# AaronZ345/StyleSinger

Hardware: NVIDIA H100
Metric: mel_frames_per_sec_ph2wav_T100 (higher is better)
Workload: dtype f32

## Files before the change

stylesinger_b200/csrc/conv_gemm_tc.cu:

```cuda
#include <cuda_fp16.h>
#include <stdlib.h>
#include <string.h>

#include <atomic>
#include <mutex>
#include <unordered_map>

#include "conv_gemm_tc.cuh"
#include "tc_common.cuh"

namespace ssb {

namespace {

constexpr int BM = 128, BK = 64;
constexpr int A_TILE = BM * BK * 2;
constexpr int EPI_WARPS = 8;
constexpr int NTHREADS = 128 + 32 * EPI_WARPS;
constexpr int XPOSE_BYTES = EPI_WARPS * 32 * 32 * 4;

constexpr int HALO = 8;
constexpr int A3_ROWS = BM + 2 * HALO;
constexpr int A3_TILE = A3_ROWS * BK * 2;
constexpr int ASLOTS = 2;

template <int BN, bool REUSE>
struct Cfg {
  static constexpr int B_TILE = BN * BK * 2;
  static constexpr int STAGE = REUSE ? 2 * B_TILE : 2 * A_TILE + 2 * B_TILE;
  static constexpr int STAGES = BN == 128 ? 3 : 4;
  static constexpr int ARING = REUSE ? ASLOTS * 2 * A3_TILE : 0;
  static constexpr int SMEM = ARING + STAGES * STAGE + XPOSE_BYTES + 1024 + 256;
  static_assert(SMEM <= 227 * 1024, "exceeds the 227 KB of shared memory a Hopper block can have");
};

struct TCParams {
  const int2* tiles;
  int ntiles, NT, taps, kchunks, dil, center, N;
  EpiTC e;
};

using namespace tc;


struct Pre {
  float4 a[8];
};

template <int MODE>
__device__ __forceinline__ void prefetch_chunk(const EpiTC& e, int64_t r0, int nrows, int n, int lane, Pre& p, int tq) {
  (void)nrows;
  if (e.n_valid > 0 && n >= e.n_valid) return;
  const int rq = lane >> 3, q4 = (lane & 7) * 4;
  const float* src = nullptr;
  int64_t st = 0;
  bool once = false;
  if constexpr (MODE == EPI_GENERIC) {
    if (!e.res) return;
    src = e.res + (r0 + rq) * e.ld_res + n + q4; st = 4 * (int64_t)e.ld_res;
  } else if constexpr (MODE == EPI_RES_SKIP) {
    if (n < e.C) {
      if (e.rh) {
        const __half* ph = e.rh + (r0 + rq) * e.ld_rh + n + q4;
        const __half* pl = e.rl + (r0 + rq) * e.ld_rh + n + q4;
        const int64_t sth = 4 * (int64_t)e.ld_rh;
#pragma unroll
        for (int i = 0; i < 8; ++i, ph += sth, pl += sth) {
          const uint2 h = *reinterpret_cast<const uint2*>(ph);
          const uint2 l = *reinterpret_cast<const uint2*>(pl);
          p.a[i] = make_float4(__uint_as_float(h.x), __uint_as_float(h.y), __uint_as_float(l.x), __uint_as_float(l.y));
        }
        return;
      }
      src = e.res + (r0 + rq) * e.ld_res + n + q4; st = 4 * (int64_t)e.ld_res;
    } else if (!e.skip_init) {
      if (e.skip_tiled) {
        src = e.skip + ((int64_t)tq * (e.C >> 5) + ((n - e.C) >> 5)) * 1024 + rq * 32 + q4; st = 128;
      } else {
        src = e.skip + (r0 + rq) * e.ld_skip + (n - e.C) + q4; st = 4 * (int64_t)e.ld_skip;
      }
      once = true;
    } else return;
  } else {
    if (!e.add) return;
    src = e.add + (r0 + rq) * e.ld_add + n + q4; st = 4 * (int64_t)e.ld_add;
    once = true;
  }
  if (once) {
#pragma unroll
    for (int i = 0; i < 8; ++i, src += st) p.a[i] = __ldcs(reinterpret_cast<const float4*>(src));
  } else {
#pragma unroll
    for (int i = 0; i < 8; ++i, src += st) p.a[i] = *reinterpret_cast<const float4*>(src);
  }
}

__device__ __forceinline__ void split_pack4(float a, float b, float c, float d, uint2& uh, uint2& ul) {
  const __half2 h0 = __floats2half2_rn(a, b), h1 = __floats2half2_rn(c, d);
  const float2 f0 = __half22float2(h0), f1 = __half22float2(h1);
  const __half2 l0 = __floats2half2_rn(a - f0.x, b - f0.y), l1 = __floats2half2_rn(c - f1.x, d - f1.y);
  uh.x = *reinterpret_cast<const uint32_t*>(&h0); uh.y = *reinterpret_cast<const uint32_t*>(&h1);
  ul.x = *reinterpret_cast<const uint32_t*>(&l0); ul.y = *reinterpret_cast<const uint32_t*>(&l1);
}
__device__ __forceinline__ void split_pack2(float a, float b, uint32_t& uh, uint32_t& ul) {
  const __half2 h0 = __floats2half2_rn(a, b);
  const float2 f0 = __half22float2(h0);
  const __half2 l0 = __floats2half2_rn(a - f0.x, b - f0.y);
  uh = *reinterpret_cast<const uint32_t*>(&h0);
  ul = *reinterpret_cast<const uint32_t*>(&l0);
}
__device__ __forceinline__ float act_slope_of(int act, float slope) {
  return act == ACT_RELU ? 0.0f : (act == ACT_LRELU ? slope : 1.0f);
}
template <int MODE>
__device__ __forceinline__ void epilogue_chunk(const EpiTC& e, const float4* xb, int64_t r0, int nrows, int n, int lane,
                                               const Pre& pre, int tq) {
  if (e.n_valid > 0 && n >= e.n_valid) return;
  const int q = lane & 7, rq = lane >> 3;
  const int n4 = n + 4 * q;
  const int64_t rb = r0 + rq;
  const float4* xr = xb + rq * 8;
  const int qx = q ^ rq;
  float b0 = 0.f, b1 = 0.f, b2 = 0.f, b3 = 0.f;
  if (e.bias) {
    const float4 bv = __ldg(reinterpret_cast<const float4*>(e.bias + n4));
    b0 = bv.x; b1 = bv.y; b2 = bv.z; b3 = bv.w;
  }
  const int nsteps = nrows > rq ? (nrows - rq + 3) >> 2 : 0;
  if constexpr (MODE == EPI_GATE) {
    const int64_t st = 4 * (int64_t)e.ldh;
    __half* ph = e.oh + rb * e.ldh + (n4 >> 1);
    __half* pl = e.ol + rb * e.ldh + (n4 >> 1);
    const bool has_add = e.add != nullptr;
#pragma unroll
    for (int i = 0; i < 8; ++i, ph += st, pl += st) {
      const float4 acc = xr[i * 32 + (qx ^ (4 * (i & 1)))];
      float g0 = acc.x + b0, f0 = acc.y + b1, g1 = acc.z + b2, f1 = acc.w + b3;
      if (has_add) {
        const float4 ad = pre.a[i];
        g0 += ad.x; f0 += ad.y; g1 += ad.z; f1 += ad.w;
      }
      uint32_t zh, zl;
      split_pack2(gate_act(g0, f0), gate_act(g1, f1), zh, zl);
      if (i < nsteps) {
        *reinterpret_cast<uint32_t*>(ph) = zh;
        *reinterpret_cast<uint32_t*>(pl) = zl;
      }
    }
  } else if constexpr (MODE == EPI_RES_SKIP) {
    if (n < e.C) {
      const float beta = e.beta;
      float s0 = 0.f, s1 = 0.f, s2 = 0.f, s3 = 0.f;
      const bool planes = e.oh != nullptr;
      if (planes && e.vec2) {
        const float4 sv = __ldg(reinterpret_cast<const float4*>(e.vec2 + n4));
        s0 = sv.x; s1 = sv.y; s2 = sv.z; s3 = sv.w;
      }
      const bool res_planes = e.rh != nullptr, has_out = e.out != nullptr;
      float c0 = 0.f, c1 = 0.f, c2 = 0.f, c3 = 0.f;
      if (res_planes && e.vec1) {
        const float4 cv = __ldg(reinterpret_cast<const float4*>(e.vec1 + n4));
        c0 = cv.x; c1 = cv.y; c2 = cv.z; c3 = cv.w;
      }
      float* po = has_out ? e.out + rb * e.ldo + n4 : nullptr;
      const int64_t sto = 4 * (int64_t)e.ldo, sth = 4 * (int64_t)e.ldh;
      __half* ph = planes ? e.oh + rb * e.ldh + n4 : nullptr;
      __half* pl = planes ? e.ol + rb * e.ldh + n4 : nullptr;
#pragma unroll
      for (int i = 0; i < 8; ++i) {
        const float4 acc = xr[i * 32 + (qx ^ (4 * (i & 1)))];
        float4 x0 = pre.a[i];
        if (res_planes) {
          const uint32_t u0 = __float_as_uint(x0.x), u1 = __float_as_uint(x0.y), u2 = __float_as_uint(x0.z), u3 = __float_as_uint(x0.w);
          const float2 h01 = __half22float2(*reinterpret_cast<const __half2*>(&u0)), h23 = __half22float2(*reinterpret_cast<const __half2*>(&u1));
          const float2 l01 = __half22float2(*reinterpret_cast<const __half2*>(&u2)), l23 = __half22float2(*reinterpret_cast<const __half2*>(&u3));
          x0 = make_float4((h01.x + l01.x) - c0, (h01.y + l01.y) - c1, (h23.x + l23.x) - c2, (h23.y + l23.y) - c3);
        }
        const float v0 = (acc.x + b0 + x0.x) * beta, v1 = (acc.y + b1 + x0.y) * beta;
        const float v2 = (acc.z + b2 + x0.z) * beta, v3 = (acc.w + b3 + x0.w) * beta;
        uint2 yh, yl;
        split_pack4(v0 + s0, v1 + s1, v2 + s2, v3 + s3, yh, yl);
        const bool ok = i < nsteps;
        if (ok && has_out) *reinterpret_cast<float4*>(po) = make_float4(v0, v1, v2, v3);
        if (ok && planes) {
          *reinterpret_cast<uint2*>(ph) = yh;
          *reinterpret_cast<uint2*>(pl) = yl;
        }
        po += sto; ph += sth; pl += sth;
      }
    } else {
      const int sc = n4 - e.C;
      const bool init = e.skip_init != 0;
      const bool planes = e.sh != nullptr;
      float* ps = e.skip_tiled ? e.skip + ((int64_t)tq * (e.C >> 5) + ((n - e.C) >> 5)) * 1024 + rq * 32 + 4 * q
                               : e.skip + rb * e.ld_skip + sc;
      const int64_t sts = e.skip_tiled ? 128 : 4 * (int64_t)e.ld_skip, sth = 4 * (int64_t)e.C;
      __half* ph = planes ? e.sh + rb * e.C + sc : nullptr;
      __half* pl = planes ? e.sl + rb * e.C + sc : nullptr;
#pragma unroll
      for (int i = 0; i < 8; ++i) {
        const float4 acc = xr[i * 32 + (qx ^ (4 * (i & 1)))];
        float v0 = acc.x + b0, v1 = acc.y + b1, v2 = acc.z + b2, v3 = acc.w + b3;
        if (!init) {
          const float4 o = pre.a[i];
          v0 += o.x; v1 += o.y; v2 += o.z; v3 += o.w;
        }
        const bool ok = i < nsteps;
        if (ok) __stcs(reinterpret_cast<float4*>(ps), make_float4(v0, v1, v2, v3));
        if (planes) {
          uint2 kh, kl;
          split_pack4(v0, v1, v2, v3, kh, kl);
          if (ok) {
            *reinterpret_cast<uint2*>(ph) = kh;
            *reinterpret_cast<uint2*>(pl) = kl;
          }
        }
        ps += sts; ph += sth; pl += sth;
      }
    }
  } else {
    const float sa = act_slope_of(e.act, e.act_slope), sp = act_slope_of(e.plane_act, e.plane_slope);
    const bool gelu = e.act == ACT_GELU;
    const float alpha = e.alpha;
    const float* rmask = e.rowmask ? e.rowmask + rb : nullptr;
    const bool has_res = e.res != nullptr, has_out = e.out != nullptr, accum = e.accum != 0, planes = e.oh != nullptr;
    const float gamma = e.gamma;
    float s0 = 0.f, s1 = 0.f, s2 = 0.f, s3 = 0.f;
    if (planes && e.vec2) {
      const float4 sv = __ldg(reinterpret_cast<const float4*>(e.vec2 + n4));
      s0 = sv.x; s1 = sv.y; s2 = sv.z; s3 = sv.w;
    }
    float* po = has_out ? e.out + rb * e.ldo + n4 : nullptr;
    int64_t sto = 4 * (int64_t)e.ldo;
    const int64_t sth = 4 * (int64_t)e.ldh;
    if (has_out && e.out_nb > 0) {
      const int blk = n4 / e.out_nb;
      po = e.out + (int64_t)blk * e.out_bs + rb * e.out_nb + (n4 - blk * e.out_nb);
      sto = 4 * (int64_t)e.out_nb;
    }
    __half* ph = planes ? e.oh + rb * e.ldh + n4 : nullptr;
    __half* pl = planes ? e.ol + rb * e.ldh + n4 : nullptr;
    float4 oacc[8];
    if (has_out && accum) {
      const float* pr = po;
#pragma unroll
      for (int i = 0; i < 8; ++i, pr += sto) oacc[i] = *reinterpret_cast<const float4*>(pr);
    }
#pragma unroll
    for (int i = 0; i < 8; ++i) {
      const float4 acc = xr[i * 32 + (qx ^ (4 * (i & 1)))];
      float v0 = (acc.x + b0) * alpha, v1 = (acc.y + b1) * alpha, v2 = (acc.z + b2) * alpha, v3 = (acc.w + b3) * alpha;
      if (gelu) {
        v0 = gelu_erf(v0); v1 = gelu_erf(v1); v2 = gelu_erf(v2); v3 = gelu_erf(v3);
      } else {
        v0 = fmaxf(v0, v0 * sa); v1 = fmaxf(v1, v1 * sa); v2 = fmaxf(v2, v2 * sa); v3 = fmaxf(v3, v3 * sa);
      }
      if (has_res) {
        const float4 x0 = pre.a[i];
        v0 += x0.x; v1 += x0.y; v2 += x0.z; v3 += x0.w;
      }
      if (rmask) {
        const float mk = rmask[4 * i];
        v0 *= mk; v1 *= mk; v2 *= mk; v3 *= mk;
      }
      if (has_out && accum) {
        const float4 o = oacc[i];
        v0 = (v0 + o.x) * gamma; v1 = (v1 + o.y) * gamma; v2 = (v2 + o.z) * gamma; v3 = (v3 + o.w) * gamma;
      }
      const bool ok = i < nsteps;
      if (ok && has_out) *reinterpret_cast<float4*>(po) = make_float4(v0, v1, v2, v3);
      if (planes) {
        const float w0 = v0 + s0, w1 = v1 + s1, w2 = v2 + s2, w3 = v3 + s3;
        uint2 qh, ql;
        split_pack4(fmaxf(w0, w0 * sp), fmaxf(w1, w1 * sp), fmaxf(w2, w2 * sp), fmaxf(w3, w3 * sp), qh, ql);
        if (ok) {
          *reinterpret_cast<uint2*>(ph) = qh;
          *reinterpret_cast<uint2*>(pl) = ql;
        }
      }
      po += sto; ph += sth; pl += sth;
    }
  }
}

template <int BN, int CL, int MODE, bool REUSE>
__global__ void __launch_bounds__(NTHREADS, 1)
conv_gemm_wg_kernel(const __grid_constant__ CUtensorMap tmA_hi, const __grid_constant__ CUtensorMap tmA_lo,
                    const __grid_constant__ CUtensorMap tmB_hi, const __grid_constant__ CUtensorMap tmB_lo,
                    const TCParams p) {
  using K = Cfg<BN, REUSE>;
  constexpr int STAGES = K::STAGES;
  constexpr int HB = BN / CL;
  constexpr int NCH = BN / 32;
  extern __shared__ uint8_t smem_raw[];
  uint8_t* smem = reinterpret_cast<uint8_t*>((reinterpret_cast<uintptr_t>(smem_raw) + 1023) & ~uintptr_t(1023));
  float* xpose = reinterpret_cast<float*>(smem + K::ARING + STAGES * K::STAGE);
  uint64_t* bars = reinterpret_cast<uint64_t*>(smem + K::ARING + STAGES * K::STAGE + XPOSE_BYTES);
  const uint32_t abase = smem_u32(smem), sbase = abase + K::ARING;
  const uint32_t full0 = smem_u32(bars), empty0 = full0 + 8 * STAGES, afull0 = empty0 + 8 * STAGES, aempty0 = afull0 + 8 * ASLOTS;
  const int warp = threadIdx.x >> 5, lane = threadIdx.x & 31;
  const uint32_t rank = CL > 1 ? cluster_rank() : 0u;
  const int cid = (int)blockIdx.x / CL, ncl = (int)gridDim.x / CL;

  if (threadIdx.x == 0) {
    for (int s = 0; s < STAGES; ++s) {
      mbar_init(full0 + 8 * s, 1);
      mbar_init(empty0 + 8 * s, CL * EPI_WARPS);
    }
    for (int s = 0; s < ASLOTS; ++s) {
      mbar_init(afull0 + 8 * s, 1);
      mbar_init(aempty0 + 8 * s, EPI_WARPS);
    }
    asm volatile("fence.mbarrier_init.release.cluster;" ::: "memory");
  }
  if (CL > 1) cluster_sync_all();
  else __syncthreads();

  const int total = (CL > 1 ? (p.ntiles + 1) / 2 : p.ntiles) * p.NT;
  const int nk = p.taps * p.kchunks;

  if (warp < 4) {
    asm volatile("setmaxnreg.dec.sync.aligned.u32 40;\n" ::: "memory");
    if (warp == 0 && lane == 0) {
      int stage = 0, as = 0;
      uint32_t phase = 0, aph = 0;
      auto load_b = [&](const CUtensorMap* mb_h, const CUtensorMap* mb_l, int c0, int brow, uint32_t extra_bytes) {
        mbar_wait(empty0 + 8 * stage, phase ^ 1);
        const uint32_t fb = full0 + 8 * stage;
        mbar_expect_tx(fb, 2 * K::B_TILE + extra_bytes);
        const uint32_t sb = sbase + stage * K::STAGE + (REUSE ? 0u : (uint32_t)(2 * A_TILE));
        if (CL > 1) {
          const uint32_t boff = rank * (uint32_t)(HB * BK * 2);
          tma_load_2d_mc(sb + boff, mb_h, fb, c0, brow + (int)rank * HB, (uint16_t)3);
          tma_load_2d_mc(sb + K::B_TILE + boff, mb_l, fb, c0, brow + (int)rank * HB, (uint16_t)3);
        } else {
          tma_load_2d(sb, mb_h, fb, c0, brow);
          tma_load_2d(sb + K::B_TILE, mb_l, fb, c0, brow);
        }
        return fb;
      };
      for (int tile = cid; tile < total; tile += ncl) {
        const int mq = tile / p.NT, nt = tile - mq * p.NT;
        int mt = CL * mq + (int)rank;
        if (mt >= p.ntiles) mt = CL * mq;
        const int row0 = p.tiles[mt].x;
        if constexpr (REUSE) {
          for (int kc = 0; kc < p.kchunks; ++kc) {
            mbar_wait(aempty0 + 8 * as, aph ^ 1);
            const uint32_t ab = afull0 + 8 * as, sa = abase + as * (2 * A3_TILE);
            mbar_expect_tx(ab, 2 * A3_TILE);
            tma_load_2d(sa, &tmA_hi, ab, kc * BK, row0 - HALO);
            tma_load_2d(sa + A3_TILE, &tmA_lo, ab, kc * BK, row0 - HALO);
            if (++as == ASLOTS) { as = 0; aph ^= 1; }
            for (int tap = 0; tap < 3; ++tap) {
              load_b(&tmB_hi, &tmB_lo, kc * BK, tap * p.N + nt * BN, 0u);
              if (++stage == STAGES) { stage = 0; phase ^= 1; }
            }
          }
        } else {
          for (int kb = 0; kb < nk; ++kb) {
            const int tap = kb / p.kchunks;
            const int c0 = (kb - tap * p.kchunks) * BK;
            const int arow = row0 + (tap - p.center) * p.dil;
            const uint32_t fb = load_b(&tmB_hi, &tmB_lo, c0, tap * p.N + nt * BN, (uint32_t)(2 * A_TILE));
            const uint32_t sa = sbase + stage * K::STAGE;
            tma_load_2d(sa, &tmA_hi, fb, c0, arow);
            tma_load_2d(sa + A_TILE, &tmA_lo, fb, c0, arow);
            if (++stage == STAGES) { stage = 0; phase ^= 1; }
          }
        }
      }
    }
    __syncwarp();
  } else {
    asm volatile("setmaxnreg.inc.sync.aligned.u32 232;\n" ::: "memory");
    const int cw = (warp - 4) >> 2;
    const int ew = (warp - 4) >> 1;
    const int eg = warp & 1;
    float* xb_pair = xpose + ew * 2048;
    const uint32_t pair_bar = 1u + (uint32_t)ew;
    const uint32_t peer_empty0 = CL > 1 ? mapa_u32(empty0, rank ^ 1u) : 0u;
    int stage = 0, as = 0;
    uint32_t phase = 0, aph = 0;
    float acc[BN / 2];
    auto release_b = [&](int st) {
      __syncwarp();
      if (lane == 0) {
        mbar_arrive(empty0 + 8 * st);
        if (CL > 1) mbar_arrive_cluster(peer_empty0 + 8 * st);
      }
    };
    auto mma_block = [&](uint64_t dah, uint64_t dal, uint64_t dbh, uint64_t dbl) {
      wg_fence();
      fence_acc(acc);
#pragma unroll
      for (int ks = 0; ks < BK / 16; ++ks) {
        const uint64_t off = (uint64_t)((ks * 32) >> 4);
        if constexpr (BN == 128) {
          wgmma_n128(acc, dah + off, dbh + off, 1u);
          wgmma_n128(acc, dah + off, dbl + off, 1u);
          wgmma_n128(acc, dal + off, dbh + off, 1u);
        } else {
          wgmma_n64(acc, dah + off, dbh + off, 1u);
          wgmma_n64(acc, dah + off, dbl + off, 1u);
          wgmma_n64(acc, dal + off, dbh + off, 1u);
        }
      }
      wg_commit();
      fence_acc(acc);
      wg_wait<1>();
      fence_acc(acc);
    };
    for (int tile = cid; tile < total; tile += ncl) {
      const int mq = tile / p.NT, nt = tile - mq * p.NT;
      const int mt = CL * mq + (int)rank;
      const int2 t = mt < p.ntiles ? p.tiles[mt] : make_int2(0, 0);
      const int64_t r0 = (int64_t)t.x + ew * 32;
      const int nrows = min(32, max(0, t.y - ew * 32));
      const int tq = mt * 4 + ew;
      const int n0 = nt * BN;
      Pre cur, nxt;
      if (nrows > 0) prefetch_chunk<MODE>(p.e, r0, nrows, n0 + eg * 32, lane, cur, tq);
#pragma unroll
      for (int i = 0; i < BN / 2; ++i) acc[i] = 0.f;
      int prev = -1;
      if constexpr (REUSE) {
        for (int kc = 0; kc < p.kchunks; ++kc) {
          mbar_wait(afull0 + 8 * as, aph);
          const uint32_t sa = abase + as * (2 * A3_TILE) + cw * 8192;
          for (int tap = 0; tap < 3; ++tap) {
            mbar_wait(full0 + 8 * stage, phase);
            const uint32_t sb = sbase + stage * K::STAGE;
            const uint32_t sh = (uint32_t)(HALO + (tap - 1) * p.dil) * 128u;
            mma_block(make_sdesc(sa + sh), make_sdesc(sa + A3_TILE + sh), make_sdesc(sb), make_sdesc(sb + K::B_TILE));
            if (prev >= 0) release_b(prev);
            prev = stage;
            if (++stage == STAGES) { stage = 0; phase ^= 1; }
          }
          wg_wait<0>();
          fence_acc(acc);
          release_b(prev);
          prev = -1;
          __syncwarp();
          if (lane == 0) mbar_arrive(aempty0 + 8 * as);
          if (++as == ASLOTS) { as = 0; aph ^= 1; }
        }
      } else {
        for (int kb = 0; kb < nk; ++kb) {
          mbar_wait(full0 + 8 * stage, phase);
          const uint32_t sa = sbase + stage * K::STAGE;
          mma_block(make_sdesc(sa + cw * 8192), make_sdesc(sa + A_TILE + cw * 8192), make_sdesc(sa + 2 * A_TILE),
                    make_sdesc(sa + 2 * A_TILE + K::B_TILE));
          if (prev >= 0) release_b(prev);
          prev = stage;
          if (++stage == STAGES) { stage = 0; phase ^= 1; }
        }
        wg_wait<0>();
        fence_acc(acc);
        if (prev >= 0) release_b(prev);
      }
      const int rbase = 16 * (warp & 1) + (lane >> 2);
#pragma unroll
      for (int cp = 0; cp < BN / 64; ++cp) {
#pragma unroll
        for (int nb = 0; nb < 8; ++nb) {
          float* xb = xb_pair + (nb >> 2) * 1024;
          const int cc = 8 * (nb & 3) + 2 * (lane & 3);
#pragma unroll
          for (int h = 0; h < 2; ++h) {
            const int rr = rbase + 8 * h;
            const int j = 4 * (8 * cp + nb) + 2 * h;
            *reinterpret_cast<float2*>(xb + (rr * 8 + ((cc >> 2) ^ (rr & 7))) * 4 + (cc & 3)) = make_float2(acc[j], acc[j + 1]);
          }
        }
        named_sync(pair_bar, 64);
        const int ch = 2 * cp + eg;
        if (ch + 2 < NCH && nrows > 0) prefetch_chunk<MODE>(p.e, r0, nrows, n0 + (ch + 2) * 32, lane, nxt, tq);
        if (nrows > 0)
          epilogue_chunk<MODE>(p.e, reinterpret_cast<float4*>(xb_pair + eg * 1024), r0, nrows, n0 + ch * 32, lane, cur, tq);
        cur = nxt;
        named_sync(pair_bar, 64);
      }
    }
  }
  if (CL > 1) cluster_sync_all();
}

__global__ void k_split_planes(const float* x, int ld, int64_t rows, int C, float scale, __half* hi, __half* lo) {
  const int64_t i = (int64_t)blockIdx.x * blockDim.x + threadIdx.x;
  if (i >= rows * C) return;
  const int64_t r = i / C;
  const int c = (int)(i - r * C);
  const float v = x[r * ld + c] * scale;
  const __half h = __float2half_rn(v);
  hi[i] = h;
  lo[i] = __float2half_rn(v - __half2float(h));
}

typedef CUresult (*EncodeTiledFn)(CUtensorMap*, CUtensorMapDataType, cuuint32_t, void*, const cuuint64_t*, const cuuint64_t*,
                                  const cuuint32_t*, const cuuint32_t*, CUtensorMapInterleave, CUtensorMapSwizzle,
                                  CUtensorMapL2promotion, CUtensorMapFloatOOBfill);
std::mutex g_host_mu;

EncodeTiledFn get_encode() {
  static std::atomic<EncodeTiledFn> fn_cached{nullptr};
  static std::atomic<bool> tried{false};
  if (!tried.load(std::memory_order_acquire)) {
    std::lock_guard<std::mutex> lk(g_host_mu);
    if (!tried.load(std::memory_order_relaxed)) {
      void* fn = nullptr;
      cudaDriverEntryPointQueryResult q;
      if (cudaGetDriverEntryPoint("cuTensorMapEncodeTiled", &fn, cudaEnableDefault, &q) == cudaSuccess &&
          q == cudaDriverEntryPointSuccess)
        fn_cached.store((EncodeTiledFn)fn, std::memory_order_relaxed);
      tried.store(true, std::memory_order_release);
    }
  }
  return fn_cached.load(std::memory_order_relaxed);
}

int make_map(CUtensorMap* m, const void* ptr, uint64_t rows, uint64_t cols, uint32_t box_rows) {
  EncodeTiledFn enc = get_encode();
  SSB_CHECK(enc != nullptr, "cuTensorMapEncodeTiled unavailable");
  cuuint64_t dims[2] = {cols, rows};
  cuuint64_t strides[1] = {cols * sizeof(__half)};
  cuuint32_t box[2] = {(cuuint32_t)BK, box_rows};
  cuuint32_t es[2] = {1, 1};
  CUresult rc = enc(m, CU_TENSOR_MAP_DATA_TYPE_FLOAT16, 2, const_cast<void*>(ptr), dims, strides, box, es,
                    CU_TENSOR_MAP_INTERLEAVE_NONE, CU_TENSOR_MAP_SWIZZLE_128B, CU_TENSOR_MAP_L2_PROMOTION_L2_256B,
                    CU_TENSOR_MAP_FLOAT_OOB_FILL_NONE);
  SSB_CHECK(rc == CUDA_SUCCESS, "cuTensorMapEncodeTiled failed");
  return 0;
}

struct MapKey {
  const void* ptr; uint64_t rows; uint32_t cols, box;
  bool operator==(const MapKey& o) const { return ptr == o.ptr && rows == o.rows && cols == o.cols && box == o.box; }
};
struct MapKeyHash {
  size_t operator()(const MapKey& k) const {
    uint64_t h = (uint64_t)(uintptr_t)k.ptr * 0x9E3779B97F4A7C15ull;
    h ^= (k.rows + 0x7F4A7C15u) * 0xC2B2AE3D27D4EB4Full;
    h ^= ((uint64_t)k.cols << 32 | k.box) * 0x165667B19E3779F9ull;
    return (size_t)(h ^ (h >> 29));
  }
};
std::unordered_map<MapKey, CUtensorMap, MapKeyHash> g_map_cache;
long long g_map_encodes = 0, g_map_hits = 0;

int cached_act_map(CUtensorMap* m, const void* ptr, uint64_t rows, uint64_t cols, uint32_t box_rows) {
  const MapKey k{ptr, rows, (uint32_t)cols, box_rows};
  std::lock_guard<std::mutex> lk(g_host_mu);
  auto it = g_map_cache.find(k);
  if (it != g_map_cache.end()) {
    *m = it->second;
    ++g_map_hits;
    return 0;
  }
  if (g_map_cache.size() > 8192) g_map_cache.clear();
  if (make_map(m, ptr, rows, cols, box_rows)) return -1;
  g_map_cache.emplace(k, *m);
  ++g_map_encodes;
  return 0;
}

constexpr int MAX_DEV = 64;
int current_device() {
  int dev = 0;
  cudaGetDevice(&dev);
  return dev >= 0 && dev < MAX_DEV ? dev : 0;
}
int device_sms() {
  static std::atomic<int> sms[MAX_DEV];
  const int dev = current_device();
  int n = sms[dev].load(std::memory_order_relaxed);
  if (n == 0) {
    cudaDeviceGetAttribute(&n, cudaDevAttrMultiProcessorCount, dev);
    if (n <= 0) n = 132;
    sms[dev].store(n, std::memory_order_relaxed);
  }
  return n;
}
template <typename KernelT>
int configure_once(KernelT kernel, std::atomic<bool>* done , int smem) {
  const int dev = current_device();
  if (done[dev].load(std::memory_order_acquire)) return 0;
  std::lock_guard<std::mutex> lk(g_host_mu);
  if (!done[dev].load(std::memory_order_relaxed)) {
    SSB_CUDA(cudaFuncSetAttribute(kernel, cudaFuncAttributeMaxDynamicSharedMemorySize, smem));
    done[dev].store(true, std::memory_order_release);
  }
  return 0;
}

struct VariantCounter { const char* name; std::atomic<long long> n; };
VariantCounter g_variants[48];
std::atomic<int> g_nvariants{0};
std::atomic<long long>* variant_counter(const char* name) {
  std::lock_guard<std::mutex> lk(g_host_mu);
  const int n = g_nvariants.load();
  for (int i = 0; i < n; ++i)
    if (strcmp(g_variants[i].name, name) == 0) return &g_variants[i].n;
  if (n >= 48) return &g_variants[47].n;
  g_variants[n].name = name;
  g_variants[n].n.store(0);
  g_nvariants.store(n + 1);
  return &g_variants[n].n;
}
const char* mode_name(int mode) { return mode == EPI_GATE ? "GATE" : (mode == EPI_RES_SKIP ? "RES_SKIP" : "GENERIC"); }

constexpr int map_index(int rows) { return rows == 64 ? 0 : 1; }
std::mutex g_pair_mu;
cudaEvent_t g_pair_evt[MAX_DEV];
cudaStream_t g_pair_last_stream[MAX_DEV];
bool g_pair_evt_valid[MAX_DEV];
void pair_guard_begin(int dev, cudaStream_t st) {
  if (!g_pair_evt[dev] && cudaEventCreateWithFlags(&g_pair_evt[dev], cudaEventDisableTiming) != cudaSuccess) {
    g_pair_evt[dev] = nullptr;
    return;
  }
  if (g_pair_evt_valid[dev] && g_pair_last_stream[dev] != st) cudaStreamWaitEvent(st, g_pair_evt[dev], 0);
}
void pair_guard_end(int dev, cudaStream_t st) {
  if (!g_pair_evt[dev]) return;
  g_pair_evt_valid[dev] = cudaEventRecord(g_pair_evt[dev], st) == cudaSuccess;
  g_pair_last_stream[dev] = st;
}

template <int BN, int CL, int MODE, bool REUSE>
int launch_m(Ctx& ctx, const GemmTC& p, TCParams tp, int num_sms) {
  using KCfg = Cfg<BN, REUSE>;
  static std::atomic<bool> configured[MAX_DEV];
  if (configure_once(conv_gemm_wg_kernel<BN, CL, MODE, REUSE>, configured, KCfg::SMEM)) return -2;
  static std::atomic<long long>* const counter = [] {
    static char name[48];
    if (CL > 1) snprintf(name, sizeof(name), "tc2%s<%d,%s>", REUSE ? "r" : "", BN / 2, mode_name(MODE));
    else snprintf(name, sizeof(name), "tc%s<%d,%s>", REUSE ? "r" : "", BN, mode_name(MODE));
    return variant_counter(name);
  }();
  const ConvTC& w = *p.w;
  const int bi = map_index(BN / CL);
  const uint32_t a_rows = REUSE ? A3_ROWS : BM;
  CUtensorMap ta_hi, ta_lo;
  if (cached_act_map(&ta_hi, p.A_hi, (uint64_t)p.rows_total, (uint64_t)w.Cin, a_rows)) return -1;
  if (cached_act_map(&ta_lo, p.A_lo, (uint64_t)p.rows_total, (uint64_t)w.Cin, a_rows)) return -1;
  tp.NT = w.N / BN;
  const int total = (CL > 1 ? (tp.ntiles + 1) / 2 : tp.ntiles) * tp.NT;
  const int slots = num_sms / CL;
  const int ncl = total < slots ? total : slots;
  cudaLaunchConfig_t cfg;
  memset(&cfg, 0, sizeof(cfg));
  cfg.gridDim = dim3((unsigned)(CL * ncl));
  cfg.blockDim = dim3(NTHREADS);
  cfg.dynamicSmemBytes = KCfg::SMEM;
  cfg.stream = ctx.stream;
  cudaLaunchAttribute at[1];
  at[0].id = cudaLaunchAttributeClusterDimension;
  at[0].val.clusterDim.x = (unsigned)CL; at[0].val.clusterDim.y = 1; at[0].val.clusterDim.z = 1;
  cfg.attrs = at; cfg.numAttrs = 1;
  {
    const bool guard = CL > 1;
    const int dev = guard ? current_device() : 0;
    std::unique_lock<std::mutex> lk(g_pair_mu, std::defer_lock);
    if (guard) {
      lk.lock();
      pair_guard_begin(dev, ctx.stream);
    }
    const cudaError_t le =
        cudaLaunchKernelEx(&cfg, conv_gemm_wg_kernel<BN, CL, MODE, REUSE>, ta_hi, ta_lo, w.tm_hi[bi], w.tm_lo[bi], tp);
    if (guard) pair_guard_end(dev, ctx.stream);
    SSB_CUDA(le);
  }
  ++g_launches;
  counter->fetch_add(1, std::memory_order_relaxed);
  return 0;
}
template <int BN, int CL>
int launch(Ctx& ctx, const GemmTC& p, const TCParams& tp, int num_sms) {
  switch (tp.e.mode) {
    case EPI_GATE: return launch_m<BN, CL, EPI_GATE, false>(ctx, p, tp, num_sms);
    case EPI_RES_SKIP: return launch_m<BN, CL, EPI_RES_SKIP, false>(ctx, p, tp, num_sms);
    default: return launch_m<BN, CL, EPI_GENERIC, false>(ctx, p, tp, num_sms);
  }
}
bool tap_reuse_eligible(const GemmTC& p, const ConvTC& w) {
  return w.taps == 3 && w.center == 1 && w.dil >= 1 && w.dil <= HALO && (p.e.mode == EPI_GATE || p.e.mode == EPI_GENERIC);
}

}

bool tc_available() { return get_encode() != nullptr; }
int make_act_map(CUtensorMap* m, const void* ptr, int64_t rows, int cols, int box_rows) {
  return cached_act_map(m, ptr, (uint64_t)rows, (uint64_t)cols, (uint32_t)box_rows);
}
long long variant_launch_count(const char* name) {
  const int n = g_nvariants.load();
  for (int i = 0; i < n; ++i)
    if (strcmp(g_variants[i].name, name) == 0) return g_variants[i].n.load();
  return 0;
}
int variant_names(char* buf, int cap) {
  int o = 0;
  const int n = g_nvariants.load();
  for (int i = 0; i < n; ++i) {
    const int l = (int)strlen(g_variants[i].name);
    if (o + l + 2 > cap) break;
    memcpy(buf + o, g_variants[i].name, l);
    o += l;
    buf[o++] = ';';
  }
  if (cap > 0) buf[o < cap ? o : cap - 1] = 0;
  return n;
}
void tensor_map_cache_stats(long long* encodes, long long* hits) {
  std::lock_guard<std::mutex> lk(g_host_mu);
  *encodes = g_map_encodes;
  *hits = g_map_hits;
}

int make_weight_maps(ConvTC* w) {
  SSB_CHECK(w->Cin % BK == 0 && w->N % 64 == 0, "tensor-core path needs Cin % 64 == 0 and N % 64 == 0");
  if (make_map(&w->tm_hi[0], w->W_hi, (uint64_t)w->taps * w->N, (uint64_t)w->Cin, 64)) return -1;
  if (make_map(&w->tm_lo[0], w->W_lo, (uint64_t)w->taps * w->N, (uint64_t)w->Cin, 64)) return -1;
  if (make_map(&w->tm_hi[1], w->W_hi, (uint64_t)w->taps * w->N, (uint64_t)w->Cin, 32)) return -1;
  if (make_map(&w->tm_lo[1], w->W_lo, (uint64_t)w->taps * w->N, (uint64_t)w->Cin, 32)) return -1;
  w->hb = w->N % 128 == 0 ? 64 : 32;
  w->ok = true;
  return 0;
}

int conv_gemm_tc(Ctx& ctx, const GemmTC& p) {
  if (ctx.dry || p.ntiles == 0) return 0;
  const ConvTC& w = *p.w;
  SSB_CHECK(w.ok, "conv_gemm_tc: weights not packed for the tensor-core path");
  SSB_CHECK(p.e.act == ACT_NONE || p.e.act == ACT_RELU || p.e.act == ACT_LRELU || p.e.act == ACT_GELU,
            "conv_gemm_tc: unsupported epilogue activation");
  SSB_CHECK(p.e.plane_act == ACT_NONE || p.e.plane_act == ACT_LRELU, "conv_gemm_tc: unsupported plane activation");
  SSB_CHECK(p.e.mode != EPI_GENERIC || p.e.out || p.e.oh, "conv_gemm_tc: GENERIC epilogue without an output");
  SSB_CHECK(p.e.mode != EPI_RES_SKIP || p.e.res || (p.e.rh && p.e.rl), "conv_gemm_tc: RES_SKIP epilogue without a residual source");
  const int num_sms = device_sms();
  TCParams tp;
  tp.tiles = p.tiles; tp.ntiles = p.ntiles; tp.taps = w.taps; tp.kchunks = w.Cin / BK;
  tp.dil = w.dil; tp.center = w.center; tp.N = w.N; tp.e = p.e;
  if (!tp.e.bias) tp.e.bias = w.bias;
  if ((int64_t)((p.ntiles + 1) / 2) * (w.N / (2 * w.hb)) >= (int64_t)num_sms) {
    if (tap_reuse_eligible(p, w)) {
      if (p.e.mode == EPI_GATE) return w.hb == 64 ? launch_m<128, 2, EPI_GATE, true>(ctx, p, tp, num_sms) : launch_m<64, 2, EPI_GATE, true>(ctx, p, tp, num_sms);
      return w.hb == 64 ? launch_m<128, 2, EPI_GENERIC, true>(ctx, p, tp, num_sms) : launch_m<64, 2, EPI_GENERIC, true>(ctx, p, tp, num_sms);
    }
    return w.hb == 64 ? launch<128, 2>(ctx, p, tp, num_sms) : launch<64, 2>(ctx, p, tp, num_sms);
  }
  return launch<64, 1>(ctx, p, tp, num_sms);
}

int split_planes(Ctx& ctx, const float* x, int ld, int64_t rows, int C, float scale, __half* hi, __half* lo) {
  if (ctx.dry || rows == 0) return 0;
  const int64_t n = rows * C;
  k_split_planes<<<(unsigned)((n + 255) / 256), 256, 0, ctx.stream>>>(x, ld, rows, C, scale, hi, lo);
  SSB_CUDA(cudaGetLastError());
  ++g_launches;
  return 0;
}

}
```

stylesinger_b200/csrc/tc_common.cuh:

```cuda
#pragma once
#include <cuda.h>
#include <cuda_fp16.h>
#include <stdint.h>

#include "common.cuh"

namespace ssb {
namespace tc {

__device__ __forceinline__ uint32_t smem_u32(const void* p) { return (uint32_t)__cvta_generic_to_shared(p); }

__device__ __forceinline__ void mbar_init(uint32_t bar, uint32_t count) {
  asm volatile("mbarrier.init.shared::cta.b64 [%0], %1;" ::"r"(bar), "r"(count) : "memory");
}
__device__ __forceinline__ void mbar_expect_tx(uint32_t bar, uint32_t bytes) {
  asm volatile("mbarrier.arrive.expect_tx.shared::cta.b64 _, [%0], %1;" ::"r"(bar), "r"(bytes) : "memory");
}
__device__ __forceinline__ void mbar_arrive(uint32_t bar) {
  asm volatile("mbarrier.arrive.shared::cta.b64 _, [%0];" ::"r"(bar) : "memory");
}
__device__ __forceinline__ void mbar_wait(uint32_t bar, uint32_t parity) {
  uint32_t done = 0;
  const long long t0 = clock64();
  while (true) {
    asm volatile(
        "{\n.reg .pred p;\nmbarrier.try_wait.parity.shared::cta.b64 p, [%1], %2;\nselp.u32 %0, 1, 0, p;\n}\n"
        : "=r"(done)
        : "r"(bar), "r"(parity)
        : "memory");
    if (done) break;
    if (clock64() - t0 > 4000000000LL) __trap();
  }
}
__device__ __forceinline__ void tma_load_2d(uint32_t dst, const CUtensorMap* map, uint32_t bar, int c0, int c1) {
  asm volatile(
      "cp.async.bulk.tensor.2d.shared::cluster.global.mbarrier::complete_tx::bytes [%0], [%1, {%3, %4}], [%2];"
      ::"r"(dst), "l"(map), "r"(bar), "r"(c0), "r"(c1)
      : "memory");
}
__device__ __forceinline__ void tma_load_2d_mc(uint32_t dst, const CUtensorMap* map, uint32_t bar, int c0, int c1, uint16_t mask) {
  asm volatile(
      "cp.async.bulk.tensor.2d.shared::cluster.global.mbarrier::complete_tx::bytes.multicast::cluster [%0], [%1, {%3, %4}], [%2], %5;"
      ::"r"(dst), "l"(map), "r"(bar), "r"(c0), "r"(c1), "h"(mask)
      : "memory");
}
__device__ __forceinline__ uint32_t cluster_rank() {
  uint32_t r;
  asm volatile("mov.u32 %0, %%cluster_ctarank;" : "=r"(r));
  return r;
}
__device__ __forceinline__ void cluster_sync_all() {
  asm volatile("barrier.cluster.arrive.release.aligned;\nbarrier.cluster.wait.acquire.aligned;" ::: "memory");
}
__device__ __forceinline__ uint32_t mapa_u32(uint32_t addr, uint32_t rank) {
  uint32_t r;
  asm volatile("mapa.shared::cluster.u32 %0, %1, %2;" : "=r"(r) : "r"(addr), "r"(rank));
  return r;
}
__device__ __forceinline__ void mbar_arrive_cluster(uint32_t bar_cluster) {
  asm volatile("mbarrier.arrive.release.cluster.shared::cluster.b64 _, [%0];" ::"r"(bar_cluster) : "memory");
}
__device__ __forceinline__ void named_sync(uint32_t id, uint32_t count) {
  asm volatile("bar.sync %0, %1;" ::"r"(id), "r"(count) : "memory");
}

__device__ __forceinline__ uint64_t make_sdesc(uint32_t saddr) {
  uint64_t d = 0;
  d |= (uint64_t)((saddr & 0x3FFFFu) >> 4);
  d |= (uint64_t)1 << 16;
  d |= (uint64_t)(1024u >> 4) << 32;
  d |= (uint64_t)1 << 62;
  return d;
}
__device__ __forceinline__ void wg_fence() { asm volatile("wgmma.fence.sync.aligned;" ::: "memory"); }
__device__ __forceinline__ void wg_commit() { asm volatile("wgmma.commit_group.sync.aligned;" ::: "memory"); }
template <int N>
__device__ __forceinline__ void wg_wait() { asm volatile("wgmma.wait_group.sync.aligned %0;" ::"n"(N) : "memory"); }
template <int R>
__device__ __forceinline__ void fence_acc(float (&d)[R]) {
#pragma unroll
  for (int i = 0; i < R; ++i) asm volatile("" : "+f"(d[i])::"memory");
}

__device__ __forceinline__ void wgmma_n64(float (&d)[32], uint64_t da, uint64_t db, uint32_t accum) {
  asm volatile(
      "{\n.reg .pred p;\nsetp.ne.b32 p, %34, 0;\n"
      "wgmma.mma_async.sync.aligned.m64n64k16.f32.f16.f16 {%0, %1, %2, %3, %4, %5, %6, %7, %8, %9, %10, %11, %12, %13, %14, %15, %16, %17, %18, %19, %20, %21, %22, %23, %24, %25, %26, %27, %28, %29, %30, %31}, %32, %33, p, 1, 1, 0, 0;\n}\n"
      : "+f"(d[0]), "+f"(d[1]), "+f"(d[2]), "+f"(d[3]), "+f"(d[4]), "+f"(d[5]), "+f"(d[6]), "+f"(d[7]), "+f"(d[8]), "+f"(d[9]), "+f"(d[10]), "+f"(d[11]), "+f"(d[12]), "+f"(d[13]), "+f"(d[14]), "+f"(d[15]), "+f"(d[16]), "+f"(d[17]), "+f"(d[18]), "+f"(d[19]), "+f"(d[20]), "+f"(d[21]), "+f"(d[22]), "+f"(d[23]), "+f"(d[24]), "+f"(d[25]), "+f"(d[26]), "+f"(d[27]), "+f"(d[28]), "+f"(d[29]), "+f"(d[30]), "+f"(d[31])
      : "l"(da), "l"(db), "r"(accum));
}

__device__ __forceinline__ void wgmma_n128(float (&d)[64], uint64_t da, uint64_t db, uint32_t accum) {
  asm volatile(
      "{\n.reg .pred p;\nsetp.ne.b32 p, %66, 0;\n"
      "wgmma.mma_async.sync.aligned.m64n128k16.f32.f16.f16 {%0, %1, %2, %3, %4, %5, %6, %7, %8, %9, %10, %11, %12, %13, %14, %15, %16, %17, %18, %19, %20, %21, %22, %23, %24, %25, %26, %27, %28, %29, %30, %31, %32, %33, %34, %35, %36, %37, %38, %39, %40, %41, %42, %43, %44, %45, %46, %47, %48, %49, %50, %51, %52, %53, %54, %55, %56, %57, %58, %59, %60, %61, %62, %63}, %64, %65, p, 1, 1, 0, 0;\n}\n"
      : "+f"(d[0]), "+f"(d[1]), "+f"(d[2]), "+f"(d[3]), "+f"(d[4]), "+f"(d[5]), "+f"(d[6]), "+f"(d[7]), "+f"(d[8]), "+f"(d[9]), "+f"(d[10]), "+f"(d[11]), "+f"(d[12]), "+f"(d[13]), "+f"(d[14]), "+f"(d[15]), "+f"(d[16]), "+f"(d[17]), "+f"(d[18]), "+f"(d[19]), "+f"(d[20]), "+f"(d[21]), "+f"(d[22]), "+f"(d[23]), "+f"(d[24]), "+f"(d[25]), "+f"(d[26]), "+f"(d[27]), "+f"(d[28]), "+f"(d[29]), "+f"(d[30]), "+f"(d[31]), "+f"(d[32]), "+f"(d[33]), "+f"(d[34]), "+f"(d[35]), "+f"(d[36]), "+f"(d[37]), "+f"(d[38]), "+f"(d[39]), "+f"(d[40]), "+f"(d[41]), "+f"(d[42]), "+f"(d[43]), "+f"(d[44]), "+f"(d[45]), "+f"(d[46]), "+f"(d[47]), "+f"(d[48]), "+f"(d[49]), "+f"(d[50]), "+f"(d[51]), "+f"(d[52]), "+f"(d[53]), "+f"(d[54]), "+f"(d[55]), "+f"(d[56]), "+f"(d[57]), "+f"(d[58]), "+f"(d[59]), "+f"(d[60]), "+f"(d[61]), "+f"(d[62]), "+f"(d[63])
      : "l"(da), "l"(db), "r"(accum));
}

__device__ __forceinline__ void wgmma_rs_n128(float (&d)[64], const uint32_t (&a)[4], uint64_t db, uint32_t accum) {
  asm volatile(
      "{\n.reg .pred p;\nsetp.ne.b32 p, %69, 0;\n"
      "wgmma.mma_async.sync.aligned.m64n128k16.f32.f16.f16 {%0, %1, %2, %3, %4, %5, %6, %7, %8, %9, %10, %11, %12, %13, %14, %15, %16, %17, %18, %19, %20, %21, %22, %23, %24, %25, %26, %27, %28, %29, %30, %31, %32, %33, %34, %35, %36, %37, %38, %39, %40, %41, %42, %43, %44, %45, %46, %47, %48, %49, %50, %51, %52, %53, %54, %55, %56, %57, %58, %59, %60, %61, %62, %63}, {%64, %65, %66, %67}, %68, p, 1, 1, 0;\n}\n"
      : "+f"(d[0]), "+f"(d[1]), "+f"(d[2]), "+f"(d[3]), "+f"(d[4]), "+f"(d[5]), "+f"(d[6]), "+f"(d[7]), "+f"(d[8]), "+f"(d[9]), "+f"(d[10]), "+f"(d[11]), "+f"(d[12]), "+f"(d[13]), "+f"(d[14]), "+f"(d[15]), "+f"(d[16]), "+f"(d[17]), "+f"(d[18]), "+f"(d[19]), "+f"(d[20]), "+f"(d[21]), "+f"(d[22]), "+f"(d[23]), "+f"(d[24]), "+f"(d[25]), "+f"(d[26]), "+f"(d[27]), "+f"(d[28]), "+f"(d[29]), "+f"(d[30]), "+f"(d[31]), "+f"(d[32]), "+f"(d[33]), "+f"(d[34]), "+f"(d[35]), "+f"(d[36]), "+f"(d[37]), "+f"(d[38]), "+f"(d[39]), "+f"(d[40]), "+f"(d[41]), "+f"(d[42]), "+f"(d[43]), "+f"(d[44]), "+f"(d[45]), "+f"(d[46]), "+f"(d[47]), "+f"(d[48]), "+f"(d[49]), "+f"(d[50]), "+f"(d[51]), "+f"(d[52]), "+f"(d[53]), "+f"(d[54]), "+f"(d[55]), "+f"(d[56]), "+f"(d[57]), "+f"(d[58]), "+f"(d[59]), "+f"(d[60]), "+f"(d[61]), "+f"(d[62]), "+f"(d[63])
      : "r"(a[0]), "r"(a[1]), "r"(a[2]), "r"(a[3]), "l"(db), "r"(accum));
}

__device__ __forceinline__ float ex2_approx(float x) {
  float y;
  asm("ex2.approx.ftz.f32 %0, %1;" : "=f"(y) : "f"(x));
  return y;
}
__device__ __forceinline__ float gate_act(float g, float f) {
  f = fminf(fmaxf(f, -15.0f), 15.0f);
  g = fmaxf(g, -50.0f);
  const float e2f = ex2_approx(f * 2.8853900817779268f);
  const float eg = ex2_approx(g * -1.4426950408889634f);
  return __fdividef(e2f - 1.0f, (e2f + 1.0f) * (1.0f + eg));
}

__device__ __forceinline__ void split_store16(__half* hi, __half* lo, const float* z) {
  __align__(16) __half h[16], l[16];
#pragma unroll
  for (int j = 0; j < 16; ++j) {
    h[j] = __float2half_rn(z[j]);
    l[j] = __float2half_rn(z[j] - __half2float(h[j]));
  }
  *reinterpret_cast<uint4*>(hi) = *reinterpret_cast<const uint4*>(&h[0]);
  *reinterpret_cast<uint4*>(hi + 8) = *reinterpret_cast<const uint4*>(&h[8]);
  *reinterpret_cast<uint4*>(lo) = *reinterpret_cast<const uint4*>(&l[0]);
  *reinterpret_cast<uint4*>(lo + 8) = *reinterpret_cast<const uint4*>(&l[8]);
}

__device__ __forceinline__ int frag_row(int w, int lane, int j) { return 16 * w + (lane >> 2) + 8 * ((j >> 1) & 1); }
__device__ __forceinline__ int frag_col(int lane, int j) { return 8 * (j >> 2) + 2 * (lane & 3) + (j & 1); }

}
}
```

Before: 29940.

## Ping-pong consumer warpgroups over alternating tiles to overlap epilogue with MMA

The two consumer warpgroups stop splitting each tile by rows. Each one now computes a full 128-row tile, using two accumulator sets, and they alternate tiles. Named-barrier turn-taking hands the mainloop from one warpgroup to the other, so one warpgroup's epilogue runs while the other issues wgmma. This is meant to hide epilogue latency behind tensor-core work, in exchange for doubled accumulator registers per thread, more complex stage/phase bookkeeping, and barrier counts halved to match.

```diff
diff --git a/stylesinger_b200/csrc/conv_gemm_tc.cu b/stylesinger_b200/csrc/conv_gemm_tc.cu
--- a/stylesinger_b200/csrc/conv_gemm_tc.cu
+++ b/stylesinger_b200/csrc/conv_gemm_tc.cu
@@ -300,16 +300,16 @@
   const uint32_t full0 = smem_u32(bars), empty0 = full0 + 8 * STAGES, afull0 = empty0 + 8 * STAGES, aempty0 = afull0 + 8 * ASLOTS;
   const int warp = threadIdx.x >> 5, lane = threadIdx.x & 31;
   const uint32_t rank = CL > 1 ? cluster_rank() : 0u;
-  const int cid = (int)blockIdx.x / CL, ncl = (int)gridDim.x / CL;
+  const int ncl = (int)gridDim.x / CL;
 
   if (threadIdx.x == 0) {
     for (int s = 0; s < STAGES; ++s) {
       mbar_init(full0 + 8 * s, 1);
-      mbar_init(empty0 + 8 * s, CL * EPI_WARPS);
+      mbar_init(empty0 + 8 * s, CL * 4);
     }
     for (int s = 0; s < ASLOTS; ++s) {
       mbar_init(afull0 + 8 * s, 1);
-      mbar_init(aempty0 + 8 * s, EPI_WARPS);
+      mbar_init(aempty0 + 8 * s, 4);
     }
     asm volatile("fence.mbarrier_init.release.cluster;" ::: "memory");
   }
@@ -339,7 +339,7 @@
         }
         return fb;
       };
-      for (int tile = cid; tile < total; tile += ncl) {
+      for (int tile = (int)blockIdx.x / CL; tile < total; tile += ncl) {
         const int mq = tile / p.NT, nt = tile - mq * p.NT;
         int mt = CL * mq + (int)rank;
         if (mt >= p.ntiles) mt = CL * mq;
@@ -375,14 +375,14 @@
   } else {
     asm volatile("setmaxnreg.inc.sync.aligned.u32 232;\n" ::: "memory");
     const int cw = (warp - 4) >> 2;
-    const int ew = (warp - 4) >> 1;
+    const int pp = (warp >> 1) & 1;
     const int eg = warp & 1;
-    float* xb_pair = xpose + ew * 2048;
-    const uint32_t pair_bar = 1u + (uint32_t)ew;
+    float* xb_pair = xpose + (2 * cw + pp) * 2048;
+    const uint32_t pair_bar = 1u + (uint32_t)(2 * cw + pp);
+    const uint32_t my_turn = 5u + (uint32_t)cw, other_turn = 6u - (uint32_t)cw;
     const uint32_t peer_empty0 = CL > 1 ? mapa_u32(empty0, rank ^ 1u) : 0u;
-    int stage = 0, as = 0;
-    uint32_t phase = 0, aph = 0;
-    float acc[BN / 2];
+    int kpos = cw * nk, apos = REUSE ? cw * p.kchunks : 0;
+    float acc[2][BN / 2];
     auto release_b = [&](int st) {
       __syncwarp();
       if (lane == 0) {
@@ -390,78 +390,101 @@
         if (CL > 1) mbar_arrive_cluster(peer_empty0 + 8 * st);
       }
     };
-    auto mma_block = [&](uint64_t dah, uint64_t dal, uint64_t dbh, uint64_t dbl) {
+    auto mma_block = [&](uint32_t a_hi, uint32_t a_lo, uint64_t dbh, uint64_t dbl) {
       wg_fence();
-      fence_acc(acc);
+      fence_acc(acc[0]);
+      fence_acc(acc[1]);
 #pragma unroll
       for (int ks = 0; ks < BK / 16; ++ks) {
         const uint64_t off = (uint64_t)((ks * 32) >> 4);
-        if constexpr (BN == 128) {
-          wgmma_n128(acc, dah + off, dbh + off, 1u);
-          wgmma_n128(acc, dah + off, dbl + off, 1u);
-          wgmma_n128(acc, dal + off, dbh + off, 1u);
-        } else {
-          wgmma_n64(acc, dah + off, dbh + off, 1u);
-          wgmma_n64(acc, dah + off, dbl + off, 1u);
-          wgmma_n64(acc, dal + off, dbh + off, 1u);
+#pragma unroll
+        for (int rb = 0; rb < 2; ++rb) {
+          const uint64_t dah = make_sdesc(a_hi + rb * 8192) + off, dal = make_sdesc(a_lo + rb * 8192) + off;
+          if constexpr (BN == 128) {
+            wgmma_n128(acc[rb], dah, dbh + off, 1u);
+            wgmma_n128(acc[rb], dah, dbl + off, 1u);
+            wgmma_n128(acc[rb], dal, dbh + off, 1u);
+          } else {
+            wgmma_n64(acc[rb], dah, dbh + off, 1u);
+            wgmma_n64(acc[rb], dah, dbl + off, 1u);
+            wgmma_n64(acc[rb], dal, dbh + off, 1u);
+          }
         }
       }
       wg_commit();
-      fence_acc(acc);
+      fence_acc(acc[0]);
+      fence_acc(acc[1]);
       wg_wait<1>();
-      fence_acc(acc);
+      fence_acc(acc[0]);
+      fence_acc(acc[1]);
     };
-    for (int tile = cid; tile < total; tile += ncl) {
+    const int cid = (int)blockIdx.x / CL;
+    for (int tile = cid + cw * ncl; tile < total; tile += 2 * ncl) {
       const int mq = tile / p.NT, nt = tile - mq * p.NT;
       const int mt = CL * mq + (int)rank;
       const int2 t = mt < p.ntiles ? p.tiles[mt] : make_int2(0, 0);
-      const int64_t r0 = (int64_t)t.x + ew * 32;
-      const int nrows = min(32, max(0, t.y - ew * 32));
-      const int tq = mt * 4 + ew;
       const int n0 = nt * BN;
+      auto rows_of = [&](int c, int64_t& r0, int& nrows, int& tq) {
+        const int ew = 2 * (c / (BN / 64)) + pp;
+        r0 = (int64_t)t.x + ew * 32;
+        nrows = min(32, max(0, t.y - ew * 32));
+        tq = mt * 4 + ew;
+      };
+      auto col_of = [&](int c) { return n0 + (2 * (c % (BN / 64)) + eg) * 32; };
       Pre cur, nxt;
-      if (nrows > 0) prefetch_chunk<MODE>(p.e, r0, nrows, n0 + eg * 32, lane, cur, tq);
-#pragma unroll
-      for (int i = 0; i < BN / 2; ++i) acc[i] = 0.f;
+      {
+        int64_t r0; int nrows, tq;
+        rows_of(0, r0, nrows, tq);
+        if (nrows > 0) prefetch_chunk<MODE>(p.e, r0, nrows, col_of(0), lane, cur, tq);
+      }
+#pragma unroll
+      for (int i = 0; i < BN / 2; ++i) acc[0][i] = acc[1][i] = 0.f;
+      if (tile != cid) named_sync(my_turn, 256);
+      const bool hand_on = tile + ncl < total;
       int prev = -1;
       if constexpr (REUSE) {
-        for (int kc = 0; kc < p.kchunks; ++kc) {
-          mbar_wait(afull0 + 8 * as, aph);
-          const uint32_t sa = abase + as * (2 * A3_TILE) + cw * 8192;
-          for (int tap = 0; tap < 3; ++tap) {
-            mbar_wait(full0 + 8 * stage, phase);
+        for (int kc = 0; kc < p.kchunks; ++kc, ++apos) {
+          const int as = apos % ASLOTS;
+          mbar_wait(afull0 + 8 * as, (uint32_t)(apos / ASLOTS) & 1u);
+          const uint32_t sa = abase + as * (2 * A3_TILE);
+          for (int tap = 0; tap < 3; ++tap, ++kpos) {
+            const int stage = kpos % STAGES;
+            mbar_wait(full0 + 8 * stage, (uint32_t)(kpos / STAGES) & 1u);
             const uint32_t sb = sbase + stage * K::STAGE;
             const uint32_t sh = (uint32_t)(HALO + (tap - 1) * p.dil) * 128u;
-            mma_block(make_sdesc(sa + sh), make_sdesc(sa + A3_TILE + sh), make_sdesc(sb), make_sdesc(sb + K::B_TILE));
+            mma_block(sa + sh, sa + A3_TILE + sh, make_sdesc(sb), make_sdesc(sb + K::B_TILE));
             if (prev >= 0) release_b(prev);
+            if (tap == 0 && kc > 0 && lane == 0) mbar_arrive(aempty0 + 8 * ((apos - 1) % ASLOTS));
             prev = stage;
-            if (++stage == STAGES) { stage = 0; phase ^= 1; }
           }
-          wg_wait<0>();
-          fence_acc(acc);
-          release_b(prev);
-          prev = -1;
-          __syncwarp();
-          if (lane == 0) mbar_arrive(aempty0 + 8 * as);
-          if (++as == ASLOTS) { as = 0; aph ^= 1; }
-        }
+        }
+        if (hand_on) named_arrive(other_turn, 256);
+        wg_wait<0>();
+        fence_acc(acc[0]);
+        fence_acc(acc[1]);
+        release_b(prev);
+        if (lane == 0) mbar_arrive(aempty0 + 8 * ((apos - 1) % ASLOTS));
       } else {
-        for (int kb = 0; kb < nk; ++kb) {
-          mbar_wait(full0 + 8 * stage, phase);
+        for (int kb = 0; kb < nk; ++kb, ++kpos) {
+          const int stage = kpos % STAGES;
+          mbar_wait(full0 + 8 * stage, (uint32_t)(kpos / STAGES) & 1u);
           const uint32_t sa = sbase + stage * K::STAGE;
-          mma_block(make_sdesc(sa + cw * 8192), make_sdesc(sa + A_TILE + cw * 8192), make_sdesc(sa + 2 * A_TILE),
-                    make_sdesc(sa + 2 * A_TILE + K::B_TILE));
+          mma_block(sa, sa + A_TILE, make_sdesc(sa + 2 * A_TILE), make_sdesc(sa + 2 * A_TILE + K::B_TILE));
           if (prev >= 0) release_b(prev);
           prev = stage;
-          if (++stage == STAGES) { stage = 0; phase ^= 1; }
-        }
+        }
+        if (hand_on) named_arrive(other_turn, 256);
         wg_wait<0>();
-        fence_acc(acc);
+        fence_acc(acc[0]);
+        fence_acc(acc[1]);
         if (prev >= 0) release_b(prev);
       }
+      kpos += nk;
+      if constexpr (REUSE) apos += p.kchunks;
       const int rbase = 16 * (warp & 1) + (lane >> 2);
 #pragma unroll
-      for (int cp = 0; cp < BN / 64; ++cp) {
+      for (int c = 0; c < NCH; ++c) {
+        const int rb = c / (BN / 64), cp = c % (BN / 64);
 #pragma unroll
         for (int nb = 0; nb < 8; ++nb) {
           float* xb = xb_pair + (nb >> 2) * 1024;
@@ -470,15 +493,25 @@
           for (int h = 0; h < 2; ++h) {
             const int rr = rbase + 8 * h;
             const int j = 4 * (8 * cp + nb) + 2 * h;
-            *reinterpret_cast<float2*>(xb + (rr * 8 + ((cc >> 2) ^ (rr & 7))) * 4 + (cc & 3)) = make_float2(acc[j], acc[j + 1]);
+            *reinterpret_cast<float2*>(xb + (rr * 8 + ((cc >> 2) ^ (rr & 7))) * 4 + (cc & 3)) =
+                make_float2(acc[rb][j], acc[rb][j + 1]);
           }
         }
         named_sync(pair_bar, 64);
-        const int ch = 2 * cp + eg;
-        if (ch + 2 < NCH && nrows > 0) prefetch_chunk<MODE>(p.e, r0, nrows, n0 + (ch + 2) * 32, lane, nxt, tq);
-        if (nrows > 0)
-          epilogue_chunk<MODE>(p.e, reinterpret_cast<float4*>(xb_pair + eg * 1024), r0, nrows, n0 + ch * 32, lane, cur, tq);
-        cur = nxt;
+        constexpr bool AHEAD = BN == 64;
+        int64_t r0; int nrows, tq;
+        if (AHEAD && c + 1 < NCH) {
+          rows_of(c + 1, r0, nrows, tq);
+          if (nrows > 0) prefetch_chunk<MODE>(p.e, r0, nrows, col_of(c + 1), lane, nxt, tq);
+        }
+        rows_of(c, r0, nrows, tq);
+        if (nrows > 0) epilogue_chunk<MODE>(p.e, reinterpret_cast<float4*>(xb_pair + eg * 1024), r0, nrows, col_of(c), lane, cur, tq);
+        if (AHEAD) {
+          cur = nxt;
+        } else if (c + 1 < NCH) {
+          rows_of(c + 1, r0, nrows, tq);
+          if (nrows > 0) prefetch_chunk<MODE>(p.e, r0, nrows, col_of(c + 1), lane, cur, tq);
+        }
         named_sync(pair_bar, 64);
       }
     }
diff --git a/stylesinger_b200/csrc/tc_common.cuh b/stylesinger_b200/csrc/tc_common.cuh
--- a/stylesinger_b200/csrc/tc_common.cuh
+++ b/stylesinger_b200/csrc/tc_common.cuh
@@ -62,6 +62,9 @@
 }
 __device__ __forceinline__ void named_sync(uint32_t id, uint32_t count) {
   asm volatile("bar.sync %0, %1;" ::"r"(id), "r"(count) : "memory");
+}
+__device__ __forceinline__ void named_arrive(uint32_t id, uint32_t count) {
+  asm volatile("bar.arrive %0, %1;" ::"r"(id), "r"(count) : "memory");
 }
 
 __device__ __forceinline__ uint64_t make_sdesc(uint32_t saddr) {
```

Measured after the change: 31120 (median of 6 runs). 4.0% higher.
